# igashov/DiffLinker

Measured on NVIDIA H100. Metric: molecules/sec (T=500 denoising), higher is better.
Workload: dtype f32

## Files before the change

difflinker_b200/csrc/common.cuh:

```cuda
#pragma once
#include <cuda_runtime.h>
#include <stdint.h>

namespace dl {

constexpr int H = 128;
constexpr int MAX_DIN = 32;
constexpr int MAX_XHD = 16;

constexpr int OPT_TANH = 1;
constexpr int OPT_MEAN = 2;
constexpr int OPT_SIN = 4;
constexpr int N_SIN_FREQ = 6;
constexpr int N_SIN_FEAT = 4 * N_SIN_FREQ;
__device__ __forceinline__ float sin_freq(int k) { return __int_as_float(__float_as_int(0x1.aceeap-2f) + (k << 24)); }
__device__ __forceinline__ float sin_arg(float r, int k) { return __fmul_rn(__fsqrt_rn(__fadd_rn(r, 1e-8f)), sin_freq(k)); }
__device__ __forceinline__ float radial_rn(float dx, float dy, float dz) {
  return __fadd_rn(__fadd_rn(__fmul_rn(dx, dx), __fmul_rn(dy, dy)), __fmul_rn(dz, dz));
}

__device__ __forceinline__ void chain_wait() { asm volatile("griddepcontrol.wait;" ::: "memory"); }
__device__ __forceinline__ void chain_release() { asm volatile("griddepcontrol.launch_dependents;" ::: "memory"); }

inline bool& chain_overlap_enabled() { static bool on = true; return on; }
// ... 47 lines not shown
__device__ __forceinline__ float2 silu2(float2 x) {
  return fmul2(x, sigmoid_pair_log2(fmul2(x, make_float2(-1.4426950408889634f, -1.4426950408889634f))));
}

struct EdgeMlpW {
  const float* W1a_t;
  const float* W1b_t;
  const float* b1;
  const float* wd;
  const float* w0;
  const float* W2_t;
  const float* b2;
  const void* W2_tc;
  float w2_descale;
  float wdmax, w0max;
  const void* W1_tc;
  float w1_descale;
  const float* b1_u;
  const float* wd_u;
  const float* w0_u;
  const float* we;
  const float* we_u;
};

struct GclW : EdgeMlpW {
  const float* W3_t;
  const float* b3;
  const float* W4_t;
  const float* b4;
  const void* W3_tc;
  const void* W4_tc;
  float w3_descale, w4_descale;
};

struct EqW : EdgeMlpW {
  const float* w5;
};

struct ProjW {
  const float* W1a_t;
  const float* W1b_t;
  const float* b1;
};

struct Plan {
  const int* rowidx;
  const int* colidx;
  const int* xrowidx;
  const int* nr;
  const int* nc;
  const int* nxr;
  const int4* items;
  const int* n_items;
  const int* xmols;
  const int* n_xmols;
  const int4* xitems;
  const int* n_xitems;
};

struct Geom {
  int B, N;
  int F;
  int C;
  int D;
  int graph_type;
  float norm_constant;
  float normalization_factor;
};

}
```

difflinker_b200/csrc/dl_engine.cu:

```cuda
#include <cuda_fp16.h>
#include <cuda_runtime.h>

#include <algorithm>
#include <cmath>
#include <cstdarg>
#include <cstdio>
#include <cstdlib>
#include <cstring>
#include <ctime>
#include <map>
#include <string>
#include <vector>

#include "../../include/difflinker_b200.h"
#include "kernels_simt.cuh"
#include "kernels_tc.cuh"
#include "kernels_node_tc.cuh"

using namespace dl;

static thread_local char g_err[1024] = "";
static void set_err(const char* fmt, ...) {
  va_list ap;
  va_start(ap, fmt);
  vsnprintf(g_err, sizeof(g_err), fmt, ap);
  va_end(ap);
}

#define CK(call)                                                                          \
  do {                                                                                    \
    cudaError_t _e = (call);                                                              \
    if (_e != cudaSuccess) {                                                              \
      set_err("%s:%d %s -> %s", __FILE__, __LINE__, #call, cudaGetErrorString(_e));       \
      return DL_ERR_CUDA;                                                                 \
    }                                                                                     \
  } while (0)

namespace {

struct Workspace {
  int B = 0, N = 0;
  float *nm = nullptr, *x0 = nullptr, *xa = nullptr, *xb = nullptr, *h = nullptr, *ABg = nullptr, *ABc = nullptr,
        *agg = nullptr, *z = nullptr, *ABgmax = nullptr, *ABcmax = nullptr, *eps = nullptr;
  int* cls = nullptr;
  int *nbr = nullptr, *recs = nullptr, *xrecs = nullptr, *n_recs = nullptr;
  float4 *x04 = nullptr, *xa4 = nullptr, *xb4 = nullptr;
  int *rowidx = nullptr, *colidx = nullptr, *xrowidx = nullptr, *nr = nullptr, *nc = nullptr, *nxr = nullptr,
      *n_items = nullptr, *xmols = nullptr, *n_xmols = nullptr, *n_xitems = nullptr;
  int4* items = nullptr;
  int4* xitems = nullptr;
  int* tile_ctr = nullptr;
  unsigned long long* seeds = nullptr;
  std::vector<void*> allocs;
};

struct HostStage {
  size_t cap = 0;
  char* buf = nullptr;
};

struct KernelTimes {
  bool on = false;
  struct Rec { const char* label; cudaEvent_t a, b; };
  std::vector<Rec> pending;
  std::map<std::string, std::pair<double, long>> acc;
  void begin(cudaStream_t st, const char* label) {
    if (!on) return;
    cudaStreamCaptureStatus cap = cudaStreamCaptureStatusNone;
    cudaStreamIsCapturing(st, &cap);
    if (cap != cudaStreamCaptureStatusNone) return;
    Rec r{label, nullptr, nullptr};
    cudaEventCreate(&r.a); cudaEventCreate(&r.b);
    cudaEventRecord(r.a, st);
    pending.push_back(r);
  }
  void end(cudaStream_t st) {
    if (!on || pending.empty() || pending.back().b == nullptr) return;
    cudaStreamCaptureStatus cap = cudaStreamCaptureStatusNone;
    cudaStreamIsCapturing(st, &cap);
    if (cap != cudaStreamCaptureStatusNone) return;
    cudaEventRecord(pending.back().b, st);
  }
  void collect(cudaStream_t st) {
    if (!on || pending.empty()) return;
    cudaStreamSynchronize(st);
    for (auto& r : pending) {
      float ms = 0.f;
      if (cudaEventElapsedTime(&ms, r.a, r.b) == cudaSuccess) { auto& a = acc[r.label]; a.first += ms; a.second += 1; }
      cudaEventDestroy(r.a); cudaEventDestroy(r.b);
    }
    pending.clear();
  }
  void report() {
    if (!on || acc.empty()) return;
    double tot = 0;
    for (auto& kv : acc) tot += kv.second.first;
    for (auto& kv : acc)
      fprintf(stderr, "[dl times] %-22s %6ld launches  avg %8.2f us  share %5.1f%%\n", kv.first.c_str(), kv.second.second,
              1e3 * kv.second.first / kv.second.second, 100.0 * kv.second.first / tot);
  }
};

}

// ... 126 lines not shown
  const auto& W1 = raw.at(p + "0.weight");
  const std::vector<float> wd = column(W1, H, IN1, 2 * H), w0 = column(W1, H, IN1, 2 * H + 1);
  pk.add(&w.w0, w0);
  pk.add_tc(&w.W2_tc, tc::pack_w2(raw.at(p + "2.weight"), pk.tc, &w.w2_descale));
  pk.add_tc(&w.W1_tc, tcn::pack_blocks(scaled(W1), IN1, 2, pk.tc, &w.w1_descale));
  pk.add(&w.b1_u, scaled(raw.at(p + "0.bias")));
  pk.add(&w.wd_u, scaled(wd));
  pk.add(&w.w0_u, scaled(w0));
  w.wdmax = absmax(wd); w.w0max = absmax(w0);
  if (sin_embedding) {
    const std::vector<float> we = transpose_block(W1, H, IN1, 2 * H, N_SIN_FEAT);
    pk.add(&w.we, we);
    pk.add(&w.we_u, scaled(we));
    w.wdmax = 0.f; w.w0max = 0.f;
    for (int k = 0; k < N_SIN_FEAT; ++k) w.wdmax += absmax(std::vector<float>(we.begin() + k * H, we.begin() + (k + 1) * H));
  }
}

template <typename T>
dl_status upload_blob(const std::vector<T>& host, T** dev) {
  if (*dev) cudaFree(*dev);
  *dev = nullptr;
  CK(cudaMalloc((void**)dev, std::max<size_t>(host.size(), 1) * sizeof(T)));
  CK(cudaMemcpy(*dev, host.data(), host.size() * sizeof(T), cudaMemcpyHostToDevice));
  return DL_OK;
}

template <typename T>
dl_status dev_alloc(Workspace& ws, T** p, size_t count) {
  void* q = nullptr;
  CK(cudaMalloc(&q, std::max<size_t>(count, 1) * sizeof(T)));
  ws.allocs.push_back(q);
  *p = reinterpret_cast<T*>(q);
  return DL_OK;
}

void free_workspace(Workspace& ws) {
  for (void* p : ws.allocs) cudaFree(p);
  ws = Workspace();
}

dl_status ensure_workspace(dl_engine* e, int B, int N) {
  Workspace& ws = e->ws;
  if (ws.B == B && ws.N == N) return DL_OK;
  free_workspace(ws);
  const size_t n = (size_t)B * N;
  const int xd = 3 + e->cfg.in_node_nf;
  dl_status s;
#define WSA(field, cnt) if ((s = dev_alloc(ws, &ws.field, (cnt))) != DL_OK) return s
  WSA(nm, n); WSA(x0, n * 3); WSA(xa, n * 3); WSA(xb, n * 3); WSA(h, n * H); WSA(ABg, n * 2 * H); WSA(ABc, n * 2 * H);
  WSA(agg, n * H); WSA(z, n * xd); WSA(eps, n * xd); WSA(cls, n); WSA(x04, n); WSA(xa4, n); WSA(xb4, n); WSA(ABgmax, n * 2); WSA(ABcmax, n * 2);
  WSA(rowidx, n); WSA(colidx, n); WSA(xrowidx, n); WSA(nr, B); WSA(nc, B); WSA(nxr, B); WSA(n_items, 1);
  WSA(xmols, B); WSA(n_xmols, 1); WSA(items, n); WSA(xitems, n); WSA(n_xitems, 1); WSA(tile_ctr, 64); WSA(seeds, B);
  if (e->use_tc && e->cfg.graph_type != 0) { WSA(nbr, n * N); WSA(recs, n * CUT_REC); WSA(xrecs, n * CUT_REC); WSA(n_recs, 2); }
#undef WSA
  ws.B = B; ws.N = N;
  return DL_OK;
}

Plan make_plan(const Workspace& ws) {
  Plan p;
  p.rowidx = ws.rowidx; p.colidx = ws.colidx; p.xrowidx = ws.xrowidx; p.nr = ws.nr; p.nc = ws.nc; p.nxr = ws.nxr;
  p.items = ws.items; p.n_items = ws.n_items; p.xmols = ws.xmols; p.n_xmols = ws.n_xmols;
  p.xitems = ws.xitems; p.n_xitems = ws.n_xitems;
  return p;
}

Geom make_geom(const dl_engine* e, int B, int N) {
  Geom g;
  g.B = B; g.N = N; g.F = e->cfg.in_node_nf; g.C = e->cfg.context_node_nf; g.D = e->D;
  g.graph_type = e->cfg.graph_type; g.norm_constant = e->cfg.norm_constant;
  g.normalization_factor = e->cfg.normalization_factor;
  return g;
}

#define LAUNCH_CHECK()                                                                    \
  do {                                                                                    \
    cudaError_t _e = cudaGetLastError();                                                  \
    if (_e != cudaSuccess) {                                                              \
      set_err("%s:%d kernel launch -> %s", __FILE__, __LINE__, cudaGetErrorString(_e));   \
      return DL_ERR_CUDA;                                                                 \
    }                                                                                     \
  } while (0)

dl_status build_plan(Workspace& ws, int B, int N, int graph_type, const int8_t* node_mask, const float* linker_mask,
                     const int8_t* edge_mask, int tile_edges, int max_rows, cudaStream_t st) {
  CK(cudaMemsetAsync(ws.agg, 0, (size_t)B * N * H * sizeof(float), st));
  k_plan_mol<<<B, 256, 2 * N * sizeof(int), st>>>(N, graph_type, edge_mask, node_mask, linker_mask, ws.rowidx,
                                                  ws.colidx, ws.xrowidx, ws.nr, ws.nc, ws.nxr);
  LAUNCH_CHECK();
  k_plan_items<<<1, 1, 0, st>>>(B, tile_edges, max_rows, 1, max_rows, ws.nr, ws.nc, ws.nxr, ws.items, ws.n_items, ws.xmols,
                                ws.n_xmols, ws.xitems, ws.n_xitems);
  LAUNCH_CHECK();
  return DL_OK;
}

dl_status build_forward_plan(dl_engine* e, int B, int N, const int8_t* node_mask, const float* linker_mask,
                             const int8_t* edge_mask, cudaStream_t st) {
  const dl_status s = build_plan(e->ws, B, N, e->cfg.graph_type, node_mask, linker_mask, edge_mask,
                                 e->use_tc ? tc::TN : ET, e->use_tc ? tc::MAXR : MAXR, st);
  if (s == DL_OK) e->launches += 2;
  return s;
}

struct FwdIO {
  const float* xh = nullptr; const float* t = nullptr; int t_numel = 0; float* out = nullptr;
  const int8_t* node_mask = nullptr; const float* linker_mask = nullptr; const int8_t* edge_mask = nullptr;
  const float* context = nullptr; int* nan_flags = nullptr;
  bool sampler = false; bool inpaint = false; const float* xh0 = nullptr; const float* upd_linker_mask = nullptr;
  const float* fragment_mask = nullptr; const float* noise = nullptr; float* chain = nullptr;
  NoiseRng rng{};
  int T = 0; float norm0 = 1.f, norm1 = 1.f, bias1 = 0.f;
};

ProjW proj_of(const EdgeMlpW& w) { return ProjW{w.W1a_t, w.W1b_t, w.b1}; }

EdgeArgs edge_args(const dl_engine* e, const EdgeMlpW& w, bool coord, const int8_t* edge_mask, const float* linker_mask,
                   const float* x, const float4* x4, float* x_out = nullptr, float4* x4_out = nullptr,
                   const float* w5 = nullptr) {
  const Workspace& ws = e->ws;
  const float ksc = e->use_tc ? 1.4426950408889634f : 1.0f;
  EdgeArgs ea{};
  ea.AB = coord ? ws.ABc : ws.ABg; ea.ABmax = coord ? ws.ABcmax : ws.ABgmax;
  ea.w2_descale = w.w2_descale; ea.wdmax = w.wdmax * ksc; ea.w0max = w.w0max * ksc;
  ea.x = x; ea.x0 = ws.x0; ea.x4 = x4; ea.x04 = ws.x04; ea.x4_out = x4_out;
  ea.edge_mask = edge_mask; ea.cls = ws.cls; ea.nm = ws.nm; ea.linker_mask = linker_mask;
  ea.W2_t = w.W2_t; ea.b2 = w.b2; ea.wd = e->use_tc ? w.wd_u : w.wd; ea.w0 = e->use_tc ? w.w0_u : w.w0; ea.w5 = w5;
  ea.plan = make_plan(ws); ea.agg = coord ? nullptr : ws.agg; ea.x_out = x_out; ea.nbr = ws.nbr;
  ea.recs = coord ? ws.xrecs : ws.recs;
  ea.n_recs = coord && ws.n_recs ? ws.n_recs + 1 : ws.n_recs;
  ea.coords_range = e->opts.coords_range;
  ea.we = e->use_tc ? w.we_u : w.we;
  return ea;
}

int edge_opt(const dl_engine* e, bool coord) {
  return (coord && e->opts.tanh ? OPT_TANH : 0) | (e->opts.aggregation == DL_AGGR_MEAN ? OPT_MEAN : 0) |
         (e->opts.sin_embedding ? OPT_SIN : 0);
}

struct NodeConsumer { const EdgeMlpW* w; float* AB; float* ABmax; };
int node_consumers(const dl_engine* e, int l, int s, NodeConsumer c[2]) {
  const int L = e->cfg.n_layers, S = e->cfg.inv_sublayers;
  const Workspace& ws = e->ws;
  if (s + 1 < S) { c[0] = {&e->gcl[l * S + s + 1], ws.ABg, ws.ABgmax}; return 1; }
  c[0] = {&e->eq[l], ws.ABc, ws.ABcmax};
  if (l + 1 == L) return 1;
  c[1] = {&e->gcl[(l + 1) * S], ws.ABg, ws.ABgmax};
  return 2;
}

tcn::NodeTcArgs node_tc_args(const dl_engine* e, const GclW& w, int l, int s) {
  const Workspace& ws = e->ws;
// ... 732 lines not shown
```

difflinker_b200/csrc/kernels_simt.cuh:

```cuda
#pragma once
#include <curand_kernel.h>

#include "common.cuh"

namespace dl {

__global__ void k_plan_mol(int N, int graph_type, const int8_t* __restrict__ edge_mask,
                           const int8_t* __restrict__ node_mask, const float* __restrict__ linker_mask,
                           int* __restrict__ rowidx, int* __restrict__ colidx, int* __restrict__ xrowidx,
                           int* __restrict__ nr, int* __restrict__ nc, int* __restrict__ nxr) {
  extern __shared__ int sm_plan[];
  int* rowlive = sm_plan;
  int* collive = sm_plan + N;
  const int b = blockIdx.x;
  const int tid = threadIdx.x, lane = tid & 31, warp = tid >> 5, nwarp = blockDim.x >> 5;
  for (int i = tid; i < N; i += blockDim.x) { rowlive[i] = 0; collive[i] = 0; }
  __syncthreads();
  if ((graph_type == 0 || graph_type == 4) && edge_mask != nullptr) {
    const int8_t* em = edge_mask + (size_t)b * N * N;
    for (int i = warp; i < N; i += nwarp) {
      int any = 0;
      for (int j = lane; j < N; j += 32) {
        int v = em[(size_t)i * N + j];
        if (v != 0) { any = 1; collive[j] = 1; }
      }
      any = __any_sync(0xffffffffu, any);
      if (lane == 0 && any) rowlive[i] = 1;
    }
  } else if (graph_type == 0 || graph_type == 4) {
    for (int i = tid; i < N; i += blockDim.x) { rowlive[i] = 1; collive[i] = 1; }
  } else {
    for (int i = tid; i < N; i += blockDim.x) {
      int v = node_mask[(size_t)b * N + i] != 0;
      rowlive[i] = v; collive[i] = v;
    }
  }
  __syncthreads();
  if (tid == 0) {
    int a = 0, c = 0, x = 0;
    for (int i = 0; i < N; ++i) {
      if (rowlive[i]) {
        rowidx[(size_t)b * N + a++] = i;
        if (linker_mask == nullptr || linker_mask[(size_t)b * N + i] != 0.0f) xrowidx[(size_t)b * N + x++] = i;
      }
      if (collive[i]) colidx[(size_t)b * N + c++] = i;
    }
    nr[b] = a; nc[b] = c; nxr[b] = x;
  }
}

__global__ void k_plan_items(int B, int tile_edges, int max_rows, int col_pad, int max_rows_gcl, const int* __restrict__ nr,
                             const int* __restrict__ nc, const int* __restrict__ nxr, int4* __restrict__ items,
                             int* __restrict__ n_items, int* __restrict__ xmols, int* __restrict__ n_xmols,
                             int4* __restrict__ xitems, int* __restrict__ n_xitems, int n_cta = 0,
                             int* __restrict__ cta_begin = nullptr, int* __restrict__ xcta_begin = nullptr) {
  if (threadIdx.x != 0 || blockIdx.x != 0) return;
  int cnt = 0, xc = 0, xi = 0;
  for (int b = 0; b < B; ++b) {
    int r = nr[b], c = nc[b];
    if (r > 0 && c > 0) {
      const int cp = (c + col_pad - 1) / col_pad * col_pad;
      int per = cp >= tile_edges ? 1 : tile_edges / cp;
      if (per > max_rows_gcl) per = max_rows_gcl;
      for (int r0 = 0; r0 < r; r0 += per) items[cnt++] = make_int4(b, r0, min(per, r - r0), c);
    }
    if (nxr[b] > 0 && c > 0) {
      xmols[xc++] = b;
      int per;
      if (col_pad > 1) {
        const int cp = (c + col_pad - 1) / col_pad * col_pad;
        per = cp >= tile_edges ? 1 : tile_edges / cp;
        if (per > max_rows_gcl) per = max_rows_gcl;
      } else {
        per = c >= tile_edges ? 1 : tile_edges / c;
        if (per > max_rows) per = max_rows;
      }
      for (int r0 = 0; r0 < nxr[b]; r0 += per) xitems[xi++] = make_int4(b, r0, min(per, nxr[b] - r0), c);
    }
  }
  *n_items = cnt;
  *n_xmols = xc;
  *n_xitems = xi;
  if (n_cta > 0 && cta_begin != nullptr) {
    for (int pass = 0; pass < 2; ++pass) {
      const int4* list = pass == 0 ? items : xitems;
      const int total = pass == 0 ? cnt : xi;
      int* out = pass == 0 ? cta_begin : xcta_begin;
      if (out == nullptr) continue;
      long long sum = 0;
      for (int k = 0; k < total; ++k) sum += (long long)list[k].z * ((list[k].w + col_pad - 1) / col_pad * col_pad) + 32;
      long long run = 0;
      int c = 0;
      out[0] = 0;
      for (int k = 0; k < total; ++k) {
        while (c + 1 < n_cta && run * n_cta >= (long long)(c + 1) * sum) out[++c] = k;
        run += (long long)list[k].z * ((list[k].w + col_pad - 1) / col_pad * col_pad) + 32;
      }
      while (c < n_cta) out[++c] = total;
    }
  }
}

constexpr int ACT_SILU = 0, ACT_RELU = 1;
template <int ACT>
__device__ __forceinline__ float act_f(float x) { return ACT == ACT_RELU ? fmaxf(x, 0.f) : silu_f(x); }

constexpr int NODE_TM = 32;
constexpr int LDX = 132;

template <int K>
__device__ __forceinline__ void warp_gemm_4x4(const float* __restrict__ xs, const float* __restrict__ Wt, int lane,
                                              float (&acc)[4][4]) {
#pragma unroll 2
  for (int k = 0; k < K; k += 4) {
    float4 w[4], x[4];
#pragma unroll
    for (int q = 0; q < 4; ++q) w[q] = __ldg(reinterpret_cast<const float4*>(Wt + (size_t)(k + q) * H + lane * 4));
#pragma unroll
    for (int r = 0; r < 4; ++r) x[r] = *reinterpret_cast<const float4*>(xs + r * LDX + k);
#pragma unroll
    for (int r = 0; r < 4; ++r) {
      const float xv[4] = {x[r].x, x[r].y, x[r].z, x[r].w};
#pragma unroll
      for (int q = 0; q < 4; ++q) {
        acc[r][0] = fmaf(xv[q], w[q].x, acc[r][0]);
        acc[r][1] = fmaf(xv[q], w[q].y, acc[r][1]);
        acc[r][2] = fmaf(xv[q], w[q].z, acc[r][2]);
        acc[r][3] = fmaf(xv[q], w[q].w, acc[r][3]);
      }
    }
  }
}

__device__ __forceinline__ void zero_acc(float (&acc)[4][4]) {
#pragma unroll
  for (int r = 0; r < 4; ++r)
#pragma unroll
    for (int c = 0; c < 4; ++c) acc[r][c] = 0.f;
}

__device__ __forceinline__ float warp_absmax4(const float (&v)[4]) {
  float m = fmaxf(fmaxf(fabsf(v[0]), fabsf(v[1])), fmaxf(fabsf(v[2]), fabsf(v[3])));
#pragma unroll
  for (int o = 16; o > 0; o >>= 1) m = fmaxf(m, __shfl_xor_sync(0xffffffffu, m, o));
  return m;
}

__device__ __forceinline__ void project_ab(const float* hs_warp, const ProjW& pw, float* __restrict__ AB,
                                           float* __restrict__ ABmax, int g0, int n_total, int warp, int lane) {
  float acc[4][4];
  zero_acc(acc);
  warp_gemm_4x4<H>(hs_warp, pw.W1a_t, lane, acc);
// ... 955 lines not shown
```

difflinker_b200/csrc/kernels_tc.cuh:

```cuda
#pragma once
#include <cuda_fp16.h>

#include <cmath>
#include <cstdio>
#include <type_traits>
#include <vector>

#include "../../include/difflinker_b200.h"
#include "kernels_simt.cuh"

namespace dl {
namespace tc {

constexpr bool AVAILABLE = true;
constexpr int TN = 128;
constexpr int MAXR = 32;
constexpr int KC = 16;
constexpr int W_LBO = H * 16;
constexpr int B_LBO = TN * 16 + 16;
constexpr int SBO = 128;
constexpr int W_BYTES = KC * W_LBO;
constexpr int B_BYTES = KC * B_LBO;
constexpr float F16_TARGET = 16384.0f;

// ... 134 lines not shown
#pragma unroll
  for (int ks = 0; ks < nks; ++ks) {
    const uint64_t ah = wg_desc(a_hi + ks * 2 * a_lbo, a_lbo, SBO), al = wg_desc(a_lo + ks * 2 * a_lbo, a_lbo, SBO);
    const uint64_t bh = wg_desc(b_hi + ks * b_ks_stride, b_lbo, SBO), bl = wg_desc(b_lo + ks * b_ks_stride, b_lbo, SBO);
    wgmma_m64n128k16<TRANS_B>(d, al, bh, (accumulate || ks > 0) ? 1u : 0u);
    wgmma_m64n128k16<TRANS_B>(d, ah, bl, 1u);
    wgmma_m64n128k16<TRANS_B>(d, ah, bh, 1u);
  }
}
template <int TRANS_B = 0>
__device__ __forceinline__ void gemm_3xf16(float (&d)[64], uint32_t a_hi, uint32_t a_lo, uint32_t a_lbo, uint32_t b_hi,
                                           uint32_t b_lo, uint32_t b_lbo, uint32_t b_ks_stride, int nks, bool accumulate) {
  fence_acc(d);
  wg_fence();
  mma_3xf16<TRANS_B>(d, a_hi, a_lo, a_lbo, b_hi, b_lo, b_lbo, b_ks_stride, nks, accumulate);
  wg_commit();
  wg_wait_all();
  fence_acc(d);
}

__device__ __forceinline__ void split2v(float2 v, uint32_t& hi, uint32_t& lo) {
  __half2 h = __float22half2_rn(v);
  float2 back = __half22float2(h);
  __half2 l = __float22half2_rn(fadd2(v, make_float2(-back.x, -back.y)));
  hi = *reinterpret_cast<uint32_t*>(&h);
  lo = *reinterpret_cast<uint32_t*>(&l);
}
__device__ __forceinline__ void split2(float a, float b, uint32_t& hi, uint32_t& lo) {
  __half2 h = __floats2half2_rn(a, b);
  float2 back = __half22float2(h);
  __half2 l = __floats2half2_rn(a - back.x, b - back.y);
  hi = *reinterpret_cast<uint32_t*>(&h);
  lo = *reinterpret_cast<uint32_t*>(&l);
}
__device__ __forceinline__ int gcl_row_of_edge(int e) { return 8 * ((e & 31) >> 1) + 2 * (e >> 5) + (e & 1); }
struct Tile {
  int b, nc, slot0, nrt, c0, ncc;
  bool first_chunk, last_chunk;
  const int* rows;
  int Et;
  int start;
  int node;
};

template <bool COORD>
struct TileIter {
  const int4* list;
  const int* rowlist;
  int N, wi_end, wi, rt, c0, cache_base, lane;
  int4 cache;
  __device__ TileIter(const Plan& p, int N_) : N(N_), rt(0), c0(0), cache_base(-(1 << 30)), lane(threadIdx.x & 31) {
    list = COORD ? p.xitems : p.items;
    rowlist = COORD ? p.xrowidx : p.rowidx;
    const int total = COORD ? *p.n_xitems : *p.n_items;
    const int per = total / (int)gridDim.x, extra = total % (int)gridDim.x, c = (int)blockIdx.x;
    wi = c * per + min(c, extra);
    wi_end = wi + per + (c < extra ? 1 : 0);
    cache = make_int4(0, 0, 0, 0);
  }
  __device__ bool next(Tile& t) {
    while (wi < wi_end) {
      if (wi - cache_base >= 32) {
        cache_base = wi;
        cache = list[min(wi + lane, wi_end - 1)];
      }
      const int src = wi - cache_base;
      const int b = __shfl_sync(0xffffffffu, cache.x, src), r_begin = __shfl_sync(0xffffffffu, cache.y, src);
      const int r_count = __shfl_sync(0xffffffffu, cache.z, src), nc = __shfl_sync(0xffffffffu, cache.w, src);
      int per = nc >= TN ? 1 : TN / max(nc, 1);
      if (per > MAXR) per = MAXR;
      if (rt >= r_count || nc <= 0) { wi += 1; rt = 0; c0 = 0; continue; }
      t.b = b; t.nc = nc; t.slot0 = r_begin + rt; t.nrt = min(per, r_count - rt);
      t.c0 = c0; t.ncc = min(TN, nc - c0);
      t.first_chunk = c0 == 0; t.last_chunk = c0 + TN >= nc;
      t.rows = rowlist + (size_t)b * N;
      c0 += TN;
      if (c0 >= nc) { c0 = 0; rt += per; }
      return true;
    }
    return false;
  }
};

struct RecIter {
  const int* recs;
  int n, k, G, lane, cur, nxt, chunk;
  __device__ RecIter(const int* recs_, const int* n_recs) : recs(recs_), lane(threadIdx.x & 31), cur(0), chunk(0) {
    n = *n_recs; G = (int)gridDim.x; k = (int)blockIdx.x;
    nxt = k < n ? recs[(size_t)k * CUT_REC + lane] : 0;
  }
  __device__ bool next(Tile& t) {
    if (chunk == 0) {
      if (k >= n) return false;
      cur = nxt;
      const int kn = k + G;
      nxt = kn < n ? recs[(size_t)kn * CUT_REC + lane] : 0;
    }
    const int w1 = __shfl_sync(0xffffffffu, cur, 1), v2 = __shfl_sync(0xffffffffu, cur, 2);
    const int info = __shfl_sync(0xffffffffu, cur, (4 + lane) & 31);
    t.b = __shfl_sync(0xffffffffu, cur, 0);
    t.nc = 0; t.slot0 = 0; t.rows = nullptr;
    if (((w1 >> 8) & 1) == 0) {
      t.nrt = w1 & 0xff; t.Et = v2; t.ncc = v2; t.c0 = 0; t.first_chunk = true; t.last_chunk = true;
      t.node = info & 0xffff; t.start = info >> 16;
      k += G;
    } else {
      const int deg = v2, c0 = chunk * TN;
      t.nrt = 1; t.Et = min(TN, deg - c0); t.ncc = t.Et; t.c0 = c0;
      t.first_chunk = chunk == 0; t.last_chunk = c0 + TN >= deg;
      t.node = __shfl_sync(0xffffffffu, cur, 4) & 0xffff;
      t.start = lane == 0 ? 0 : t.Et;
      ++chunk;
      if (t.last_chunk) { chunk = 0; k += G; }
    }
    return true;
  }
};

template <bool COORD, bool SPARSE>
__device__ __forceinline__ typename std::conditional<SPARSE, RecIter, TileIter<COORD>>::type make_iter(const EdgeArgs& a, int N) {
  if constexpr (SPARSE) return RecIter(a.recs, a.n_recs);
  else return TileIter<COORD>(a.plan, N);
}

template <bool COORD, bool SPARSE = false, int OPT = 0>
__global__ void __launch_bounds__(EDGE_TC_THREADS, 1) k_edge_tc(Geom gm, EdgeArgs a, const __half* __restrict__ w2tc) {
  constexpr bool MEAN = (OPT & OPT_MEAN) != 0, TANH = (OPT & OPT_TANH) != 0, EMB = (OPT & OPT_SIN) != 0;
  static_assert(COORD || !TANH, "tanh only bounds the coordinate update");
  extern __shared__ uint8_t smem_raw[];
  uint8_t* sm = smem_raw + ((1024u - (smem_u32(smem_raw) & 1023u)) & 1023u);
  const uint32_t sbase = smem_u32(sm);
  const int tid = threadIdx.x, lane = tid & 31, warp = tid >> 5;
  const int N = gm.N;

  const uint32_t bars = sbase + OFF_BAR;
  float2* b2w5 = reinterpret_cast<float2*>(sm + OFF_B2W5);

  if (tid == 0) {
    mbar_init(bars + BAR_W, 1);
    for (int i = 0; i < N_STAGE; ++i) { mbar_init(bars + BAR_FULL + 8 * i, N_PROD_WARPS); mbar_init(bars + BAR_EMPTY + 8 * i, N_EPI_WARPS); }
    for (int i = 0; i < N_ACC; ++i) {
      mbar_init(bars + BAR_TBL + 8 * i, 1);
      mbar_init(bars + BAR_TEMPTY + 8 * i, N_EPI_WARPS);
    }
    fence_barrier_init();
  }
  if (tid < H) b2w5[tid] = make_float2(a.b2[tid], COORD ? a.w5[tid] : 0.f);
  __syncthreads();

  if (warp >= W_LOAD && warp < W_PROD) {
    asm volatile("setmaxnreg.dec.sync.aligned.u32 %0;" ::"n"(REGS_CTRL));
  if (warp >= W_TBL && warp < W_TBL + N_TBL_WARPS) {
    const int tw = warp - W_TBL;
    typename std::conditional<SPARSE, RecIter, TileIter<COORD>>::type iter = make_iter<COORD, SPARSE>(a, N);
    Tile cur;
    for (int t = 0;; ++t) {
      const int acc = t & (N_ACC - 1);
      const bool more = iter.next(cur);
      if (t % N_TBL_WARPS != tw) { if (!more) break; continue; }
      if (t >= N_ACC) mbar_wait_relaxed(bars + BAR_TEMPTY + 8 * acc, ((t - N_ACC) / N_ACC) & 1);
      uint8_t* tb = sm + OFF_TBL + acc * TBL_BYTES;
      int* hdr = reinterpret_cast<int*>(tb + TBL_HDR);
      if (more) {
        const int Et = SPARSE ? cur.Et : cur.nrt * cur.ncc;
        const size_t gb = (size_t)cur.b * N;
        int heavy_deg = 0;
        if constexpr (MEAN && SPARSE) {
          const int w1 = __shfl_sync(0xffffffffu, iter.cur, 1), v2 = __shfl_sync(0xffffffffu, iter.cur, 2);
          heavy_deg = ((w1 >> 8) & 1) ? v2 : 0;
        }
        if (lane == 0) {
          hdr[0] = Et; hdr[1] = cur.nrt; hdr[2] = cur.ncc;
          hdr[3] = (cur.first_chunk ? 1 : 0) | (cur.last_chunk ? 2 : 0);
          hdr[4] = cur.b;
          if (MEAN && SPARSE) hdr[6] = heavy_deg;
        }
        if (SPARSE) {
          if (lane < cur.nrt) {
            reinterpret_cast<int*>(tb + TBL_ROWNODE)[lane] = cur.node;
            reinterpret_cast<int*>(tb + TBL_ROWSTART)[lane] = cur.start;
          }
          if (lane == 0) reinterpret_cast<int*>(tb + TBL_ROWSTART)[cur.nrt] = Et;
        } else {
          if (lane < cur.nrt) {
            reinterpret_cast<int*>(tb + TBL_ROWNODE)[lane] = cur.rows[cur.slot0 + lane];
            reinterpret_cast<int*>(tb + TBL_ROWSTART)[lane] = lane * cur.ncc;
          }
          if (lane == 0) reinterpret_cast<int*>(tb + TBL_ROWSTART)[cur.nrt] = Et;
        }
        bool any_rescale = false;
#pragma unroll
        for (int e = lane; e < TN; e += 32) {
          const int ev = min(e, Et - 1);
          int i, j;
          float ew_list = 1.f;
          if (SPARSE) {
            int rr = 0;
            for (int r = 1; r < cur.nrt; ++r) rr += ev >= __shfl_sync(0xffffffffu, cur.start, r) ? 1 : 0;
            i = __shfl_sync(0xffffffffu, cur.node, rr);
            const int first_col = __shfl_sync(0xffffffffu, cur.start, rr);
            const int raw = a.nbr[(gb + i) * N + cur.c0 + (ev - first_col)];
            j = raw & 0x7fffffff;
            ew_list = raw < 0 ? 0.f : 1.f;
          } else {
            const int rr = ev / cur.ncc, jj = ev - rr * cur.ncc;
            i = cur.rows[cur.slot0 + rr];
            j = a.plan.colidx[gb + cur.c0 + jj];
          }
          const float4 xi = a.x4[gb + i], xj = a.x4[gb + j], yi = a.x04[gb + i], yj = a.x04[gb + j];
          const float dx = xi.x - xj.x, dy = xi.y - xj.y, dz = xi.z - xj.z;
          const float ex = yi.x - yj.x, ey = yi.y - yj.y, ez = yi.z - yj.z;
          float d, d0;
          if constexpr (EMB) {
            d = radial_rn(dx, dy, dz); d0 = radial_rn(ex, ey, ez);
          } else {
            d = dx * dx + dy * dy + dz * dz;
            d0 = ex * ex + ey * ey + ez * ez;
          }
          int ci = 0, cj = 0;
          if (!SPARSE && gm.graph_type != 0) { ci = a.cls[gb + i]; cj = a.cls[gb + j]; }
          reinterpret_cast<int*>(tb + TBL_ROWOFF)[e] = (int)((gb + i) * 2 * H);
          reinterpret_cast<int*>(tb + TBL_COLOFF)[e] = (int)((gb + j) * 2 * H + H);
          reinterpret_cast<float*>(tb + TBL_D)[e] = d;
          reinterpret_cast<float*>(tb + TBL_D0)[e] = d0;
          const float bound = EMB ? a.ABmax[(gb + i) * 2] + a.ABmax[(gb + j) * 2 + 1] + a.wdmax
                                  : a.ABmax[(gb + i) * 2] + a.ABmax[(gb + j) * 2 + 1] + d * a.wdmax + d0 * a.w0max;
          float sc = 1.0f;
          if (!(bound <= F16_TARGET)) {
            const int ex2 = ((__float_as_int(bound) >> 23) & 0xff) - 127;
            sc = __int_as_float(max(127 + 13 - ex2, 1) << 23);
          }
          reinterpret_cast<float*>(tb + TBL_SC)[e] = sc;
          any_rescale |= (sc != 1.0f);
          const float ew = SPARSE ? ew_list
                                  : edge_weight(gm.graph_type, a.edge_mask ? a.edge_mask + gb * N : nullptr, N, i, j, ci, cj, d0);
          reinterpret_cast<float2*>(tb + TBL_EM)[e] =
              COORD ? make_float2(ew, a.w2_descale / sc)
                    : make_float2(ew * -0.6931471805599453f, (a.w2_descale / sc) * -1.4426950408889634f);
          if (COORD) {
            const float inv = 1.0f / (sqrtf(d + 1e-8f) + gm.norm_constant);
            float* cds = reinterpret_cast<float*>(tb + TBL_CD);
            cds[e * 3 + 0] = dx * inv; cds[e * 3 + 1] = dy * inv; cds[e * 3 + 2] = dz * inv;
          }
        }
        any_rescale = __any_sync(0xffffffffu, any_rescale);
        if (lane == 0) hdr[5] = any_rescale ? 1 : 0;
      } else if (lane == 0) {
        hdr[0] = 0;
      }
      __syncwarp();
      if (lane == 0) mbar_arrive(bars + BAR_TBL + 8 * acc);
      if (!more) break;
    }
  } else if (warp == W_LOAD) {
    if (lane == 0) {
      mbar_expect_tx(bars + BAR_W, 2 * W_BYTES);
      bulk_g2s(sbase + OFF_WHI, w2tc, 2 * W_BYTES, bars + BAR_W);
    }
  }
  } else if (warp >= W_PROD) {
// ... 119 lines not shown
    for (int t = 0;; ++t) {
      const int acc = t & (N_ACC - 1), s = t & (N_STAGE - 1);
      if (!COORD && g == 0 && t > 0) named_sync(BAR_TURN0, 32 * N_EPI_WARPS);
      mbar_wait(bars + BAR_TBL + 8 * acc, (t / N_ACC) & 1);
      const uint8_t* tb = sm + OFF_TBL + acc * TBL_BYTES;
      const int* hdr = reinterpret_cast<const int*>(tb + TBL_HDR);
      const int Et = hdr[0];
      if (Et <= 0) break;
      const uint32_t bhi = sbase + OFF_ST + s * STAGE_BYTES, blo = bhi + B_BYTES;
      if (!COORD) {
        if (g == 1) named_sync(BAR_TURN1, 32 * N_EPI_WARPS);
        mbar_wait(bars + BAR_FULL + 8 * s, (t / N_STAGE) & 1);
        fence_acc(d);
        wg_fence();
        mma_3xf16(d, sbase + OFF_WHI + g * 1024, sbase + OFF_WLO + g * 1024, W_LBO, bhi, blo, B_LBO, 2 * B_LBO, 8, false);
        wg_commit();
        named_arrive(g == 0 ? BAR_TURN1 : BAR_TURN0, 32 * N_EPI_WARPS);
        wg_wait_all();
        fence_acc(d);
      } else {
        mbar_wait(bars + BAR_FULL + 8 * s, (t / N_STAGE) & 1);
        gemm_3xf16(d, bhi + g * 1024, blo + g * 1024, B_LBO, sbase + OFF_WHI, sbase + OFF_WLO, W_LBO, 2 * W_LBO, 8, false);
      }
      __syncwarp();
      if (lane == 0) mbar_arrive(bars + BAR_EMPTY + 8 * s);

      const int nrt = hdr[1];
      const bool first_chunk = hdr[3] & 1, last_chunk = hdr[3] & 2;
      const size_t gb = (size_t)hdr[4] * N;
      const float2* emds = reinterpret_cast<const float2*>(tb + TBL_EM);
      const int* rownode = reinterpret_cast<const int*>(tb + TBL_ROWNODE);
      const int* rowstart = reinterpret_cast<const int*>(tb + TBL_ROWSTART);
      if (!COORD) {
        const float2 bias = make_float2(b2w5[r0].x * -1.4426950408889634f, b2w5[r0 + 8].x * -1.4426950408889634f);
        const float inv_norm = 1.0f / gm.normalization_factor;
        const float inv_n = 1.0f / (float)N;
        auto put = [&](int r, float2 v) {
          float* dst = a.agg + (gb + rownode[r]) * H;
          if constexpr (MEAN) {
            const float inv = SPARSE ? rcp_approx((float)(hdr[6] > 0 ? hdr[6] : rowstart[r + 1] - rowstart[r])) : inv_n;
            dst[r0] = v.x * inv; dst[r0 + 8] = v.y * inv;
          } else {
            dst[r0] = v.x * inv_norm; dst[r0 + 8] = v.y * inv_norm;
          }
        };
        const int E0 = 32 * q;
        const bool has = E0 < Et;
        int cur = 0;
        if (has) { while (rowstart[cur + 1] <= E0) ++cur; }
        const int hrow = cur;
        uint32_t bmask = 0;
        int nr = cur + 1;
        if (has) { for (; nr <= nrt && rowstart[nr] < E0 + 32; ++nr) bmask |= 1u << (rowstart[nr] - E0); }
        const bool open_end = has && nr <= nrt && rowstart[nr] > E0 + 32;
        const bool cut = Et < E0 + 32;
        const uint32_t wmask = __reduce_or_sync(0xffffffffu, bmask);
        float2 hsum = make_float2(0.f, 0.f), sum = make_float2(0.f, 0.f);
        bool in_head = true;
#pragma unroll
        for (int tt = 0; tt < 32; ++tt) {
          if (wmask & (1u << tt)) {
            const bool here = (bmask >> tt) & 1u;
            if (here && !in_head) put(cur, sum);
            hsum = here && in_head ? sum : hsum;
            sum = here ? make_float2(0.f, 0.f) : sum;
            in_head = in_head && !here;
            cur += here ? 1 : 0;
          }
          const float2 ed = emds[E0 + tt];
          const float2 u = ffma2(make_float2(d[(tt >> 1) * 4 + (tt & 1)], d[(tt >> 1) * 4 + 2 + (tt & 1)]),
                                 make_float2(ed.y, ed.y), bias);
          const float2 v = fmul2(usig2(u), make_float2(ed.x, ed.x));
          sum = fadd2(sum, v);
        }
        if (in_head) hsum = sum;
        const float2 lsum = sum;
        const bool cont_in = has && rowstart[hrow] < E0;
        float2 cin = (q == 0 && nrt == 1 && !first_chunk) ? run : make_float2(0.f, 0.f);
#pragma unroll
        for (int k = 0; k < 3; ++k) {
          const float2 cout = in_head ? fadd2(cin, hsum) : lsum;
          const float px = __shfl_up_sync(0xffffffffu, cout.x, 1, 4), py = __shfl_up_sync(0xffffffffu, cout.y, 1, 4);
          if (q == k + 1 && cont_in) cin = make_float2(px, py);
        }
        const float2 htot = fadd2(cin, hsum);
        if (nrt == 1) {
          const int src = (lane & ~3) | ((Et - 1) >> 5);
          run = make_float2(__shfl_sync(0xffffffffu, htot.x, src), __shfl_sync(0xffffffffu, htot.y, src));
        }
        if (has && last_chunk) {
          if (!in_head || !open_end) put(hrow, htot);
          if (!in_head && !open_end && !cut) put(cur, lsum);
        }
        __syncwarp();
        if (lane == 0) mbar_arrive(bars + BAR_TEMPTY + 8 * acc);
      } else {
        const float2 eda = emds[min(r0, Et - 1)], edb = emds[min(r0 + 8, Et - 1)];
        float2 pa = make_float2(0.f, 0.f), pb = make_float2(0.f, 0.f);
#pragma unroll
        for (int j = 0; j < 16; ++j) {
          const float2 w0 = b2w5[8 * j + 2 * q], w1 = b2w5[8 * j + 2 * q + 1];
          const float2 va = ffma2(make_float2(d[4 * j], d[4 * j + 1]), make_float2(eda.y, eda.y), make_float2(w0.x, w1.x));
          const float2 vb = ffma2(make_float2(d[4 * j + 2], d[4 * j + 3]), make_float2(edb.y, edb.y), make_float2(w0.x, w1.x));
          pa = ffma2(silu2(va), make_float2(w0.y, w1.y), pa);
          pb = ffma2(silu2(vb), make_float2(w0.y, w1.y), pb);
        }
        float phia = pa.x + pa.y, phib = pb.x + pb.y;
        phia += __shfl_xor_sync(0xffffffffu, phia, 1); phib += __shfl_xor_sync(0xffffffffu, phib, 1);
        phia += __shfl_xor_sync(0xffffffffu, phia, 2); phib += __shfl_xor_sync(0xffffffffu, phib, 2);
        const float* cds = reinterpret_cast<const float*>(tb + TBL_CD);
        if constexpr (TANH) {
          const float range = a.coords_range;
          if (q == 0 && r0 < Et) {
            const float th = tanhf(phia);
#pragma unroll
            for (int k = 0; k < 3; ++k) txs[r0 * 3 + k] = cds[r0 * 3 + k] * th * range * eda.x;
          }
          if (q == 0 && r0 + 8 < Et) {
            const int e = r0 + 8;
            const float th = tanhf(phib);
#pragma unroll
            for (int k = 0; k < 3; ++k) txs[e * 3 + k] = cds[e * 3 + k] * th * range * edb.x;
          }
        } else {
          if (q == 0 && r0 < Et) {
            const float w = phia * eda.x;
            txs[r0 * 3 + 0] = cds[r0 * 3 + 0] * w; txs[r0 * 3 + 1] = cds[r0 * 3 + 1] * w; txs[r0 * 3 + 2] = cds[r0 * 3 + 2] * w;
          }
          if (q == 0 && r0 + 8 < Et) {
            const int e = r0 + 8;
            const float w = phib * edb.x;
            txs[e * 3 + 0] = cds[e * 3 + 0] * w; txs[e * 3 + 1] = cds[e * 3 + 1] * w; txs[e * 3 + 2] = cds[e * 3 + 2] * w;
          }
        }
        named_sync(2, 32 * N_EPI_WARPS);
        if (tid < nrt * 3) {
          const int rr = tid / 3, dim = tid - rr * 3;
          float sacc = (nrt == 1 && !first_chunk) ? run3 : 0.f;
          const int col0 = rowstart[rr];
          const int ncc = rowstart[rr + 1] - col0;
          for (int jj = 0; jj < ncc; ++jj) sacc += txs[(col0 + jj) * 3 + dim];
          if (nrt == 1) run3 = sacc;
          if (last_chunk) {
// ... 197 lines not shown
```

Baseline: 189.9.

## Pack dense edge tiles across row boundaries and balance items per CTA

For dense graphs on the tensor-core path, the planner now chooses rows-per-item to minimise tile count and splits each item's flattened row×column edge range into full tiles that may straddle row boundaries. A linear-partition search assigns contiguous items to CTAs so each CTA gets a near-equal number of tiles, replacing the even item-count split. The aggregation epilogue carries partial row sums across chunks so rows cut between tiles are still reduced correctly. The aim is fewer partially filled tiles and less CTA load imbalance, at the cost of a more complex serial planning kernel and carry logic.

```diff
diff --git a/difflinker_b200/csrc/common.cuh b/difflinker_b200/csrc/common.cuh
--- a/difflinker_b200/csrc/common.cuh
+++ b/difflinker_b200/csrc/common.cuh
@@ -123,6 +123,7 @@
   const int* nxr;
   const int4* items;
   const int* n_items;
+  const int* cta_begin;
   const int* xmols;
   const int* n_xmols;
   const int4* xitems;
diff --git a/difflinker_b200/csrc/dl_engine.cu b/difflinker_b200/csrc/dl_engine.cu
--- a/difflinker_b200/csrc/dl_engine.cu
+++ b/difflinker_b200/csrc/dl_engine.cu
@@ -50,6 +50,7 @@
   int4* items = nullptr;
   int4* xitems = nullptr;
   int* tile_ctr = nullptr;
+  int* cta_begin = nullptr;
   unsigned long long* seeds = nullptr;
   std::vector<void*> allocs;
 };
@@ -282,6 +283,7 @@
   WSA(agg, n * H); WSA(z, n * xd); WSA(eps, n * xd); WSA(cls, n); WSA(x04, n); WSA(xa4, n); WSA(xb4, n); WSA(ABgmax, n * 2); WSA(ABcmax, n * 2);
   WSA(rowidx, n); WSA(colidx, n); WSA(xrowidx, n); WSA(nr, B); WSA(nc, B); WSA(nxr, B); WSA(n_items, 1);
   WSA(xmols, B); WSA(n_xmols, 1); WSA(items, n); WSA(xitems, n); WSA(n_xitems, 1); WSA(tile_ctr, 64); WSA(seeds, B);
+  WSA(cta_begin, e->num_sms + 1);
   if (e->use_tc && e->cfg.graph_type != 0) { WSA(nbr, n * N); WSA(recs, n * CUT_REC); WSA(xrecs, n * CUT_REC); WSA(n_recs, 2); }
 #undef WSA
   ws.B = B; ws.N = N;
@@ -291,7 +293,7 @@
 Plan make_plan(const Workspace& ws) {
   Plan p;
   p.rowidx = ws.rowidx; p.colidx = ws.colidx; p.xrowidx = ws.xrowidx; p.nr = ws.nr; p.nc = ws.nc; p.nxr = ws.nxr;
-  p.items = ws.items; p.n_items = ws.n_items; p.xmols = ws.xmols; p.n_xmols = ws.n_xmols;
+  p.items = ws.items; p.n_items = ws.n_items; p.cta_begin = ws.cta_begin; p.xmols = ws.xmols; p.n_xmols = ws.n_xmols;
   p.xitems = ws.xitems; p.n_xitems = ws.n_xitems;
   return p;
 }
@@ -314,21 +316,22 @@
   } while (0)
 
 dl_status build_plan(Workspace& ws, int B, int N, int graph_type, const int8_t* node_mask, const float* linker_mask,
-                     const int8_t* edge_mask, int tile_edges, int max_rows, cudaStream_t st) {
+                     const int8_t* edge_mask, int tile_edges, int max_rows, cudaStream_t st, int n_cta = 0) {
   CK(cudaMemsetAsync(ws.agg, 0, (size_t)B * N * H * sizeof(float), st));
   k_plan_mol<<<B, 256, 2 * N * sizeof(int), st>>>(N, graph_type, edge_mask, node_mask, linker_mask, ws.rowidx,
                                                   ws.colidx, ws.xrowidx, ws.nr, ws.nc, ws.nxr);
   LAUNCH_CHECK();
   k_plan_items<<<1, 1, 0, st>>>(B, tile_edges, max_rows, 1, max_rows, ws.nr, ws.nc, ws.nxr, ws.items, ws.n_items, ws.xmols,
-                                ws.n_xmols, ws.xitems, ws.n_xitems);
+                                ws.n_xmols, ws.xitems, ws.n_xitems, n_cta, ws.cta_begin);
   LAUNCH_CHECK();
   return DL_OK;
 }
 
 dl_status build_forward_plan(dl_engine* e, int B, int N, const int8_t* node_mask, const float* linker_mask,
                              const int8_t* edge_mask, cudaStream_t st) {
+  const bool dense = e->use_tc && e->cfg.graph_type == 0;
   const dl_status s = build_plan(e->ws, B, N, e->cfg.graph_type, node_mask, linker_mask, edge_mask,
-                                 e->use_tc ? tc::TN : ET, e->use_tc ? tc::MAXR : MAXR, st);
+                                 e->use_tc ? tc::TN : ET, e->use_tc ? tc::MAXR : MAXR, st, dense ? e->num_sms : 0);
   if (s == DL_OK) e->launches += 2;
   return s;
 }
diff --git a/difflinker_b200/csrc/kernels_simt.cuh b/difflinker_b200/csrc/kernels_simt.cuh
--- a/difflinker_b200/csrc/kernels_simt.cuh
+++ b/difflinker_b200/csrc/kernels_simt.cuh
@@ -49,16 +49,34 @@
   }
 }
 
+__host__ __device__ __forceinline__ int dense_tile_edges(int nc, int tile_edges, int max_rows) {
+  return min(tile_edges, max_rows * nc);
+}
+constexpr int SEG_TILES = 8;
+
 __global__ void k_plan_items(int B, int tile_edges, int max_rows, int col_pad, int max_rows_gcl, const int* __restrict__ nr,
                              const int* __restrict__ nc, const int* __restrict__ nxr, int4* __restrict__ items,
                              int* __restrict__ n_items, int* __restrict__ xmols, int* __restrict__ n_xmols,
                              int4* __restrict__ xitems, int* __restrict__ n_xitems, int n_cta = 0,
-                             int* __restrict__ cta_begin = nullptr, int* __restrict__ xcta_begin = nullptr) {
+                             int* __restrict__ cta_begin = nullptr) {
   if (threadIdx.x != 0 || blockIdx.x != 0) return;
   int cnt = 0, xc = 0, xi = 0;
   for (int b = 0; b < B; ++b) {
     int r = nr[b], c = nc[b];
-    if (r > 0 && c > 0) {
+    if (r > 0 && c > 0 && n_cta > 0) {
+      const int te = dense_tile_edges(c, tile_edges, max_rows_gcl);
+      auto count = [&](int R) { return (r / R) * ((R * c + te - 1) / te) + ((r % R) * c + te - 1) / te; };
+      int per = c >= tile_edges ? 1 : tile_edges / c;
+      if (per > max_rows_gcl) per = max_rows_gcl;
+      const int base = count(per);
+      int best = per, best_t = base;
+      for (int R = 1; R <= r && (R * c + te - 1) / te <= SEG_TILES; ++R) {
+        const int t = count(R);
+        if (t < best_t) { best = R; best_t = t; }
+      }
+      if (best_t * 16 > base * 15) best = per;
+      for (int r0 = 0; r0 < r; r0 += best) items[cnt++] = make_int4(b, r0, min(best, r - r0), c);
+    } else if (r > 0 && c > 0) {
       const int cp = (c + col_pad - 1) / col_pad * col_pad;
       int per = cp >= tile_edges ? 1 : tile_edges / cp;
       if (per > max_rows_gcl) per = max_rows_gcl;
@@ -81,23 +99,33 @@
   *n_items = cnt;
   *n_xmols = xc;
   *n_xitems = xi;
-  if (n_cta > 0 && cta_begin != nullptr) {
-    for (int pass = 0; pass < 2; ++pass) {
-      const int4* list = pass == 0 ? items : xitems;
-      const int total = pass == 0 ? cnt : xi;
-      int* out = pass == 0 ? cta_begin : xcta_begin;
-      if (out == nullptr) continue;
-      long long sum = 0;
-      for (int k = 0; k < total; ++k) sum += (long long)list[k].z * ((list[k].w + col_pad - 1) / col_pad * col_pad) + 32;
-      long long run = 0;
-      int c = 0;
-      out[0] = 0;
-      for (int k = 0; k < total; ++k) {
-        while (c + 1 < n_cta && run * n_cta >= (long long)(c + 1) * sum) out[++c] = k;
-        run += (long long)list[k].z * ((list[k].w + col_pad - 1) / col_pad * col_pad) + 32;
-      }
-      while (c < n_cta) out[++c] = total;
-    }
+  if (n_cta > 0) {
+    auto tiles = [&](int k) {
+      const int4 it = items[k];
+      const int te = dense_tile_edges(it.w, tile_edges, max_rows_gcl);
+      return (it.z * it.w + te - 1) / te;
+    };
+    long long total = 0;
+    int cap = 0;
+    for (int k = 0; k < cnt; ++k) { const int t = tiles(k); total += t; cap = max(cap, t); }
+    cap = max(cap, (int)((total + n_cta - 1) / n_cta));
+    for (;; ++cap) {
+      int used = 1, fill = 0;
+      for (int k = 0; k < cnt && used <= n_cta; ++k) {
+        const int t = tiles(k);
+        if (fill + t > cap) { ++used; fill = 0; }
+        fill += t;
+      }
+      if (used <= n_cta) break;
+    }
+    int c = 0, fill = 0;
+    cta_begin[0] = 0;
+    for (int k = 0; k < cnt; ++k) {
+      const int t = tiles(k);
+      if (fill + t > cap) { cta_begin[++c] = k; fill = 0; }
+      fill += t;
+    }
+    while (c < n_cta) cta_begin[++c] = cnt;
   }
 }
 
diff --git a/difflinker_b200/csrc/kernels_tc.cuh b/difflinker_b200/csrc/kernels_tc.cuh
--- a/difflinker_b200/csrc/kernels_tc.cuh
+++ b/difflinker_b200/csrc/kernels_tc.cuh
@@ -210,10 +210,16 @@
   __device__ TileIter(const Plan& p, int N_) : N(N_), rt(0), c0(0), cache_base(-(1 << 30)), lane(threadIdx.x & 31) {
     list = COORD ? p.xitems : p.items;
     rowlist = COORD ? p.xrowidx : p.rowidx;
-    const int total = COORD ? *p.n_xitems : *p.n_items;
-    const int per = total / (int)gridDim.x, extra = total % (int)gridDim.x, c = (int)blockIdx.x;
-    wi = c * per + min(c, extra);
-    wi_end = wi + per + (c < extra ? 1 : 0);
+    const int c = (int)blockIdx.x;
+    if (COORD) {
+      const int total = *p.n_xitems;
+      const int per = total / (int)gridDim.x, extra = total % (int)gridDim.x;
+      wi = c * per + min(c, extra);
+      wi_end = wi + per + (c < extra ? 1 : 0);
+    } else {
+      wi = p.cta_begin[c];
+      wi_end = p.cta_begin[c + 1];
+    }
     cache = make_int4(0, 0, 0, 0);
   }
   __device__ bool next(Tile& t) {
@@ -225,6 +231,17 @@
       const int src = wi - cache_base;
       const int b = __shfl_sync(0xffffffffu, cache.x, src), r_begin = __shfl_sync(0xffffffffu, cache.y, src);
       const int r_count = __shfl_sync(0xffffffffu, cache.z, src), nc = __shfl_sync(0xffffffffu, cache.w, src);
+      if constexpr (!COORD) {
+        const int seg = r_count * nc;
+        if (rt >= seg || nc <= 0) { wi += 1; rt = 0; continue; }
+        const int Et = min(dense_tile_edges(nc, TN, MAXR), seg - rt), fr = rt / nc;
+        t.b = b; t.nc = nc; t.slot0 = r_begin + fr; t.nrt = (rt + Et - 1) / nc - fr + 1;
+        t.c0 = rt - fr * nc; t.ncc = Et; t.Et = Et;
+        t.first_chunk = t.c0 == 0; t.last_chunk = (rt + Et) % nc == 0;
+        t.rows = rowlist + (size_t)b * N;
+        rt += Et;
+        return true;
+      }
       int per = nc >= TN ? 1 : TN / max(nc, 1);
       if (per > MAXR) per = MAXR;
       if (rt >= r_count || nc <= 0) { wi += 1; rt = 0; c0 = 0; continue; }
@@ -320,7 +337,7 @@
       uint8_t* tb = sm + OFF_TBL + acc * TBL_BYTES;
       int* hdr = reinterpret_cast<int*>(tb + TBL_HDR);
       if (more) {
-        const int Et = SPARSE ? cur.Et : cur.nrt * cur.ncc;
+        const int Et = SPARSE || !COORD ? cur.Et : cur.nrt * cur.ncc;
         const size_t gb = (size_t)cur.b * N;
         int heavy_deg = 0;
         if constexpr (MEAN && SPARSE) {
@@ -342,7 +359,7 @@
         } else {
           if (lane < cur.nrt) {
             reinterpret_cast<int*>(tb + TBL_ROWNODE)[lane] = cur.rows[cur.slot0 + lane];
-            reinterpret_cast<int*>(tb + TBL_ROWSTART)[lane] = lane * cur.ncc;
+            reinterpret_cast<int*>(tb + TBL_ROWSTART)[lane] = COORD ? lane * cur.ncc : lane == 0 ? 0 : lane * cur.nc - cur.c0;
           }
           if (lane == 0) reinterpret_cast<int*>(tb + TBL_ROWSTART)[cur.nrt] = Et;
         }
@@ -360,10 +377,14 @@
             const int raw = a.nbr[(gb + i) * N + cur.c0 + (ev - first_col)];
             j = raw & 0x7fffffff;
             ew_list = raw < 0 ? 0.f : 1.f;
-          } else {
+          } else if (COORD) {
             const int rr = ev / cur.ncc, jj = ev - rr * cur.ncc;
             i = cur.rows[cur.slot0 + rr];
             j = a.plan.colidx[gb + cur.c0 + jj];
+          } else {
+            const int g = cur.c0 + ev, rr = g / cur.nc, jj = g - rr * cur.nc;
+            i = cur.rows[cur.slot0 + rr];
+            j = a.plan.colidx[gb + jj];
           }
           const float4 xi = a.x4[gb + i], xj = a.x4[gb + j], yi = a.x04[gb + i], yj = a.x04[gb + j];
           const float dx = xi.x - xj.x, dy = xi.y - xj.y, dz = xi.z - xj.z;
@@ -589,7 +610,7 @@
         uint32_t bmask = 0;
         int nr = cur + 1;
         if (has) { for (; nr <= nrt && rowstart[nr] < E0 + 32; ++nr) bmask |= 1u << (rowstart[nr] - E0); }
-        const bool open_end = has && nr <= nrt && rowstart[nr] > E0 + 32;
+        const bool open_end = has && ((nr <= nrt && rowstart[nr] > E0 + 32) || (!last_chunk && Et <= E0 + 32));
         const bool cut = Et < E0 + 32;
         const uint32_t wmask = __reduce_or_sync(0xffffffffu, bmask);
         float2 hsum = make_float2(0.f, 0.f), sum = make_float2(0.f, 0.f);
@@ -613,7 +634,7 @@
         if (in_head) hsum = sum;
         const float2 lsum = sum;
         const bool cont_in = has && rowstart[hrow] < E0;
-        float2 cin = (q == 0 && nrt == 1 && !first_chunk) ? run : make_float2(0.f, 0.f);
+        float2 cin = (q == 0 && !first_chunk) ? run : make_float2(0.f, 0.f);
 #pragma unroll
         for (int k = 0; k < 3; ++k) {
           const float2 cout = in_head ? fadd2(cin, hsum) : lsum;
@@ -621,11 +642,12 @@
           if (q == k + 1 && cont_in) cin = make_float2(px, py);
         }
         const float2 htot = fadd2(cin, hsum);
-        if (nrt == 1) {
+        if (!last_chunk) {
           const int src = (lane & ~3) | ((Et - 1) >> 5);
-          run = make_float2(__shfl_sync(0xffffffffu, htot.x, src), __shfl_sync(0xffffffffu, htot.y, src));
-        }
-        if (has && last_chunk) {
+          const float2 tail = in_head ? htot : lsum;
+          run = make_float2(__shfl_sync(0xffffffffu, tail.x, src), __shfl_sync(0xffffffffu, tail.y, src));
+        }
+        if (has) {
           if (!in_head || !open_end) put(hrow, htot);
           if (!in_head && !open_end && !cut) put(cur, lsum);
         }
```

Result: faster. 195.9, median of 6 (+3.2%).
